# JSybrandt/HypergraphEmbedding

Measured on AMD Instinct MI355X. Metric: training samples/sec + alg-dist SpMV GB/s, HOBE dim=128 at 1/2/4/8 MI355X, higher is better.
Workload: dtype f32; 1 GPU; C3 HG2V_ALG_DIST (HOBE) dim=128, random 100k/50k, 1 step = 1 training epoch; nodes=100000, edges=50000, nnz=1999903, records_per_epoch=59999992, batch=256, dim=128, num_neighbors=5, num_samples=200, parallelism=single GPU

## Files before the change

### hypergraphembedding_amd/csrc/hgx_ctx.hip

```cpp
#include <algorithm>
#include <cstring>
#include <vector>

#include "hgx_internal.h"

int hgx_fail(hgx_ctx *ctx, int code, const char *fmt, ...) {
  if (ctx) {
    char buf[1024];
    va_list ap;
    va_start(ap, fmt);
    vsnprintf(buf, sizeof(buf), fmt, ap);
    va_end(ap);
    ctx->err = buf;
  }
  return code;
}

int hgx_ensure(hgx_ctx *ctx, DevBuf &b, size_t bytes) {
  if (bytes == 0) bytes = 16;
  if (b.bytes >= bytes) return HGX_OK;
  if (b.p) {
    hipFree(b.p);
    b.p = nullptr;
    b.bytes = 0;
// ... 86 lines not shown
  if (!ctx) return HGX_EINVAL;
  HGX_CHECK(ctx, key, HGX_EINVAL, "null tuning key");
  const std::string k(key);
  Tuning &t = ctx->tune;
  if (k == "sample_reject_w") {
    HGX_CHECK(ctx, value >= 0, HGX_EINVAL, "sample_reject_w must be >= 0");
    t.sample_reject_w = value;
  } else if (k == "sample_mode3_shift_e") {
    HGX_CHECK(ctx, value >= -10 && value <= 10, HGX_EINVAL,
              "sample_mode3_shift_e must be in [-10, 10]");
    t.sample_mode3_shift_e = (int)value;
  } else if (k == "sample_mode3_shift") {
    HGX_CHECK(ctx, value >= -10 && value <= 10, HGX_EINVAL,
              "sample_mode3_shift must be in [-10, 10]");
    t.sample_mode3_shift = (int)value;
  } else if (k == "sample_mode3") {
    HGX_CHECK(ctx, value >= 0 && value <= 2, HGX_EINVAL, "sample_mode3 must be 0, 1 or 2");
    t.sample_mode3 = (int)value;
  } else if (k == "train_fused") {
    HGX_CHECK(ctx, value == 0 || value == 1, HGX_EINVAL, "train_fused must be 0 or 1");
    t.train_fused = (int)value;
  } else if (k == "train_lanes") {
    HGX_CHECK(ctx, value == 0 || value == 32 || value == 64, HGX_EINVAL,
              "train_lanes must be 0, 32 or 64");
    t.train_lanes = (int)value;
  } else if (k == "train_tb") {
    HGX_CHECK(ctx, value == 0 || value == 128 || value == 256 || value == 512, HGX_EINVAL,
              "train_tb must be 0, 128, 256 or 512");
    t.train_tb = (int)value;
  } else if (k == "train_wave_pair") {
    HGX_CHECK(ctx, (value >= -1 && value <= 1) || value == 3 || value == 4, HGX_EINVAL,
              "train_wave_pair must be -1, 0, 1, 3 or 4");
    t.train_wave_pair = (int)value;
  } else if (k == "alg_long") {
    HGX_CHECK(ctx, value == 0 || (value >= 64 && value <= (1 << 20)), HGX_EINVAL,
              "alg_long must be 0 or in [64, 2^20]");
    t.alg_long = (int)value;
  } else if (k == "alg_push") {
    HGX_CHECK(ctx, value == 0 || value == 1, HGX_EINVAL, "alg_push must be 0 or 1");
    t.alg_push = (int)value;
  } else if (k == "mlp_fuse_head") {
    HGX_CHECK(ctx, value == 0 || value == 1, HGX_EINVAL, "mlp_fuse_head must be 0 or 1");
    t.mlp_fuse_head = (int)value;
  } else if (k == "mlp_prefetch") {
    HGX_CHECK(ctx, value >= 0 && value <= 2, HGX_EINVAL, "mlp_prefetch must be 0, 1 or 2");
    t.mlp_prefetch = (int)value;
  } else if (k == "mlp_wgrad_split") {
    HGX_CHECK(ctx, value >= 0 && value <= 1, HGX_EINVAL, "mlp_wgrad_split must be 0 or 1");
    t.mlp_wgrad_split = (int)value;
  } else if (k == "svc_lds_m") {
    HGX_CHECK(ctx, value == 64 || value == 128 || value == 192, HGX_EINVAL,
              "svc_lds_m must be 64, 128 or 192");
    t.svc_lds_m = (int)value;
  } else if (k == "ae_chunk_rows") {
    HGX_CHECK(ctx, value >= 0 && value <= (1 << 16), HGX_EINVAL,
              "ae_chunk_rows must be in [0, 65536]");
    t.ae_chunk_rows = (int)value;
  } else if (k == "n2v_expand_w") {
    HGX_CHECK(ctx, value >= 0 && value <= (1 << 20), HGX_EINVAL,
              "n2v_expand_w must be in [0, 2^20]");
    t.n2v_expand_w = (int)value;
  } else if (k == "n2v_chunk_walks") {
    HGX_CHECK(ctx, value >= 0 && value <= (1 << 16), HGX_EINVAL,
              "n2v_chunk_walks must be in [0, 65536]");
    t.n2v_chunk_walks = (int)value;
  } else if (k == "dw_hot_levels") {
// ... 199 lines not shown
```

### hypergraphembedding_amd/csrc/hgx_internal.h

```cpp
#pragma once

#include <hip/hip_runtime.h>

#include <cstdarg>
#include <cstdint>
#include <cstdio>
#include <cstdlib>
#include <string>
#include <vector>

#include "hgx.h"

struct DevBuf {
  void *p = nullptr;
  size_t bytes = 0;
  template <class T> T *as() const { return reinterpret_cast<T *>(p); }
};

struct LongRows {
  DevBuf seg;
  DevBuf off;
  DevBuf rows;
  DevBuf part;
  int nlong = 0, nseg = 0, thresh = 0;
};
constexpr int kLongRow = 512;

struct Tuning {
  int64_t sample_reject_w = 1 << 15;
  int sample_mode3 = 0;
  int sample_mode3_shift = 1;
  int sample_mode3_shift_e = 1;
  int train_fused = 1;
  int train_lanes = 0;
  int train_tb = 0;
  int train_wave_pair = -1;
  int alg_long = 0;
  int alg_ks = 0;
  int alg_push = 0;
  int mlp_fuse_head = 1;
  int mlp_prefetch = 1;
  int mlp_wgrad_split = 0;
  int train_prep_overlap = 0;
  int train_prep_cus = 0;
  int svc_lds_m = 128;
  int ae_chunk_rows = 0;
  int n2v_expand_w = 256;
  int n2v_chunk_walks = 0;
  int dw_hot_levels = 6;
};

struct hgx_ctx {
  int device = 0;
  hipStream_t stream = nullptr;
  hipStream_t own_stream = nullptr;
  std::string err;

  int32_t N = 0, E = 0;
  int64_t nnz = 0;
  uint64_t inc_gen = 0;
  DevBuf rp_n, col_n, rp_e, col_e;
  DevBuf blk_n, blk_e;
  int nblk_n = 0, nblk_e = 0;
  LongRows long_n, long_e;
  double avg_deg_n = 0, avg_deg_e = 0;
  int32_t max_deg_n = 0, max_deg_e = 0;

  int k = 0, ks = 0;
  DevBuf X[2], Y[2];
// ... 263 lines not shown
```

### hypergraphembedding_amd/csrc/hgx_train.hip

```cpp
#include <hipcub/hipcub.hpp>

#include <algorithm>
#include <cmath>
#include <cstdlib>
#include <cstring>
#include <vector>

#include "hgx_internal.h"
#include "hgx_train_common.h"
#include "hgx_train_split.h"
#include "hgx_train_step.h"
#include "hgx_train_prep.h"
#include "hgx_train_layout.h"

namespace {

int grid_for(int64_t work, int per_block) {
  int64_t g = (work + per_block - 1) / per_block;
  return (int)std::max<int64_t>(1, std::min<int64_t>(g, 4096));
}

void geometry(int d, int &L, int &VPL) {
  const int nv = (d + 3) / 4;
  L = 1;
// ... 37 lines not shown
using KStepFn = void (*)(TrainArgs, int, int, int, int);
#endif
using KFlushFn = void (*)(TrainArgs, const int *, const int *, const int *, int, int);

template <int SL, int VW, int TB>
void step_fns(int loss, KStepFn *kf, KFlushFn &kfl) {
  kf[0] = loss == 0 ? train_step<SL, VW, 5, 1, TB, false>
                    : train_step<SL, VW, 5, 2, TB, false>;
  kf[1] = loss == 0 ? train_step<SL, VW, 5, 1, TB, true>
                    : train_step<SL, VW, 5, 2, TB, true>;
  kfl = train_flush<SL * VW / 4>;
}
#ifndef HGX_TRAIN_CHUNKWAIT
#define HGX_TRAIN_CHUNKWAIT 0
#endif
constexpr bool kMergePair4 = HGX_TRAIN_ONEKERNEL >= 1;
constexpr bool kMergeAll = HGX_TRAIN_ONEKERNEL == 2;
template <int VW>
void step_fns_pair(int loss, KStepFn *kf, KFlushFn &kfl) {
  constexpr bool M0 = kMergeAll || (kMergePair4 && VW == 4);
  kf[0] = loss == 0 ? train_step<64, VW, 5, 1, 512, M0, true>
                    : train_step<64, VW, 5, 2, 512, M0, true>;
  kf[1] = loss == 0 ? train_step<64, VW, 5, 1, 512, true, true>
                    : train_step<64, VW, 5, 2, 512, true, true>;
  kfl = train_flush<64 * VW / 4>;
}
template <int RPB>
void step_fns_quad(int loss, KStepFn *kf, KFlushFn &kfl) {
  kf[0] = loss == 0 ? train_step_q<2, 5, 1, kMergeAll, RPB> : train_step_q<2, 5, 2, kMergeAll, RPB>;
  kf[1] = loss == 0 ? train_step_q<2, 5, 1, true, RPB> : train_step_q<2, 5, 2, true, RPB>;
  kfl = train_flush<32>;
}
constexpr int kPairDefault128 = 4, kPairDefault256 = 1;
bool pick_step(int L, int VPL, int K, int loss, int act, int lanes, int pair, int &sl,
               int &tb, int &rpb, KStepFn *kf, KFlushFn &kfl) {
  if (VPL != 1 || K != 5 || loss != act) return false;
  if (L != 32 && L != 64) return false;
  const int vw = L == 32 && lanes != 32 ? 2 : 4;
  sl = L * 4 / vw;
  const int pair_auto = tb != 0 ? 0 : vw == 2 ? kPairDefault128 : kPairDefault256;
  const int form = pair < 0 ? pair_auto : pair;
  if (sl == 64 && vw == 2 && form == 3) {
    tb = 512;
    rpb = 2;
    step_fns_quad<2>(loss, kf, kfl);
    return true;
  }
  if (sl == 64 && vw == 2 && form == 4) {
    tb = 256;
    rpb = 1;
    step_fns_quad<1>(loss, kf, kfl);
    return true;
  }
  if (sl == 64 && form) {
    tb = 512;
    rpb = 4;
    if (vw == 2) step_fns_pair<2>(loss, kf, kfl);
    else step_fns_pair<4>(loss, kf, kfl);
    return true;
  }
  if (sl == 32) {
    tb = tb == 256 ? 256 : 128;
    if (tb == 128) step_fns<32, 4, 128>(loss, kf, kfl);
    else step_fns<32, 4, 256>(loss, kf, kfl);
  } else if (vw == 2) {
    tb = tb == 512 || tb == 128 ? tb : 256;
// ... 293 lines not shown
  HGX_CHECK(ctx, max_epochs >= 0, HGX_EINVAL, "epochs must be >= 0");
  HGX_CHECK(ctx, loss == 0 || loss == 1, HGX_EINVAL, "loss must be 0 or 1");
  HGX_CHECK(ctx, act == 0 || act == 1, HGX_EINVAL, "act must be 0 or 1");
  HGX_CHECK(ctx, ctx->n_rec < (int64_t)INT32_MAX, HGX_EUNSUP, "more than 2^31 records");
  HGX_HIP(ctx, hipSetDevice(ctx->device));
  const int K = ctx->K, R = 4 + 2 * K;
  HGX_CHECK(ctx, (size_t)sort_slots(batch * R) * 8 <= 64 * 1024, HGX_EUNSUP,
            "batch_size*(4+2K)=%d exceeds the 8192-slot batch limit", batch * R);
  HGX_TRY(hgx_ensure(ctx, ctx->s0, 16));
  HGX_HIP(ctx, hipMemsetAsync(ctx->s0.p, 0, 16, ctx->stream));
  hipLaunchKernelGGL(max_index, dim3(grid_for(ctx->n_rec, 256)), dim3(256), 0, ctx->stream,
                     ctx->rec_idx.as<int>(), ctx->n_rec, R, K, ctx->s0.as<int>());
  HGX_LAUNCH_CHECK(ctx);
  int mx[4] = {0, 0, 0, 0};
  HGX_HIP(ctx, hipMemcpyAsync(mx, ctx->s0.p, 16, hipMemcpyDeviceToHost, ctx->stream));
  HGX_HIP(ctx, hipStreamSynchronize(ctx->stream));
  HGX_CHECK(ctx, mx[2] == 0, HGX_EINVAL, "negative record index");
  HGX_CHECK(ctx, mx[0] < ctx->node_rows && mx[1] < ctx->edge_rows, HGX_EINVAL,
            "record index (node %d, edge %d) outside the tables (%lld, %lld)",
            mx[0], mx[1], (long long)ctx->node_rows, (long long)ctx->edge_rows);
  return HGX_OK;
}

struct TrainPlan : hgx_layout::Dims {
  int64_t n, nbatches, nchunks;
  int K, SB, P, L, VPL;
  float lr, eps;
  int loss, act;
  int tb1, tb2, grid2;
  KFn k1 = nullptr, k2 = nullptr;
  KStepFn kf[2] = {nullptr, nullptr};
  KFlushFn kfl = nullptr;
  int tbf, lstride;
  bool ahead;
  size_t prep_smem, place_smem;
  int chunk_batches(int64_t c) const { return (int)std::min<int64_t>(CB, nbatches - c * CB); }
};

static int plan_split(hgx_ctx *ctx, TrainPlan &p) {
  p.tb1 = env_int("HGX_TRAIN_TB1", p.L >= 64 ? 512 : kTB);
  if (p.tb1 != 512) p.tb1 = kTB;
  if (!(p.K == 5 && p.loss == p.act) || env_int("HGX_TRAIN_GENERIC", 0) == 1) p.tb1 = kTB;
  p.tb2 = env_int("HGX_TRAIN_TB2", 512);
  if (p.tb2 != 512) p.tb2 = kTB;
  HGX_CHECK(ctx, pick_kernels(p.L, p.VPL, p.K, p.loss, p.act, p.tb1, p.tb2, p.k1, p.k2),
            HGX_EUNSUP, "no kernel for d=%d", ctx->d);
  p.RPB = p.tb1 / p.L;
  p.nblk1 = (p.batch + p.RPB - 1) / p.RPB;
  const int GPB2 = p.tb2 / p.L;
  p.grid2 = (p.SB + GPB2 - 1) / GPB2 + 2;
  return HGX_OK;
}

static int train_plan(hgx_ctx *ctx, int batch, float lr, float eps, int loss, int act,
                      TrainPlan &p) {
  p.n = ctx->n_rec;
  p.batch = batch, p.K = ctx->K, p.R = 4 + 2 * p.K, p.dp = ctx->dp, p.r0slots = kR0Slots;
  p.lr = lr, p.eps = eps, p.loss = loss, p.act = act;
  p.SB = batch * p.R;
  p.P = sort_slots(p.SB);
  geometry(ctx->d, p.L, p.VPL);
  HGX_TRY(plan_split(ctx, p));
  p.tbf = ctx->tune.train_tb;
  int SL = 0, rpbf = 0;
  p.fused = ctx->tune.train_fused && env_int("HGX_TRAIN_GENERIC", 0) != 1 && batch <= kPackB &&
            pick_step(p.L, p.VPL, p.K, loss, act, ctx->tune.train_lanes,
                      ctx->tune.train_wave_pair, SL, p.tbf, rpbf, p.kf, p.kfl);
  p.prpb = p.fused ? rpbf : 0;
  p.NBF = p.fused ? (batch + p.prpb - 1) / p.prpb : 0;
  p.RW = p.R + kWX;
  p.Mmax = p.SB / 2 + 1;
  p.MX = p.fused ? 2 + p.Mmax : 0;
  HGX_CHECK(ctx, p.MX <= (int)kDefMask + 1, HGX_EUNSUP, "batch too large for the step");
  const bool r0e = HGX_TRAIN_R0EARLY && p.fused && ctx->dp == 2 * SL;
  p.lstride = std::max(p.nblk1, r0e ? p.NBF * p.prpb : p.NBF);
  p.nbatches = (p.n + batch - 1) / batch;
  p.CB = (int)std::min<int64_t>(1024, (p.nbatches + kChunkRound - 1) / kChunkRound * kChunkRound);
  p.nchunks = (p.nbatches + p.CB - 1) / p.CB;
  p.overlap = p.fused && ctx->tune.train_prep_overlap >= 1;
  p.ahead = p.overlap && ctx->tune.train_prep_overlap == 2;
  p.prep_smem = p.P == kSortP ? ((size_t)p.P * 8 + std::max<size_t>(kPrepB * 4, (size_t)p.SB * 2) + 15) / 16 * 16
                              : (size_t)p.P * 12 + kPrepB * 4;
  p.place_smem = sizeof(int) * ((size_t)p.Mmax + p.SB);
  return HGX_OK;
}

struct TrainTrace {
  static constexpr int kBatches = 256;
  static constexpr size_t kBytes = sizeof(unsigned long long) * kBatches * 2 * 1024 * 8;
  const char *path = nullptr;
  void *p = nullptr;
  int begin(hgx_ctx *ctx) {
    path = hgx_debug_env_str("HGX_TRAIN_TRACE");
    if (path && path[0]) {
      HGX_HIP(ctx, hipMalloc(&p, kBytes));
      HGX_HIP(ctx, hipMemset(p, 0, kBytes));
    }
#ifdef HGX_DEBUG_KNOBS
    const int ab = env_int("HGX_TRAIN_ABLATE", 0), tn = p ? kBatches : 0;
    HGX_HIP(ctx, hipMemcpyToSymbol(HIP_SYMBOL(g_tab), &ab, sizeof(int)));
    HGX_HIP(ctx, hipMemcpyToSymbol(HIP_SYMBOL(g_trace), &p, sizeof(p)));
    HGX_HIP(ctx, hipMemcpyToSymbol(HIP_SYMBOL(g_trace_nb), &tn, sizeof(tn)));
#endif
    return HGX_OK;
  }
  void write_out() const {
    std::vector<unsigned long long> h(p ? kBytes / 8 : 0);
    if (!p || hipMemcpy(h.data(), p, kBytes, hipMemcpyDeviceToHost) != hipSuccess) return;
// ... 127 lines not shown
      }
      hbrk = ctx->train_hbrk;
    }
    if (p.overlap && !p.ahead) {
      HGX_TRY(train_streams(ctx, ctx->tune.train_prep_cus));
      sst = ctx->tstream[0];
      spr = ctx->tstream[1];
    }
    bev.assign(2 * p.nchunks, nullptr);
    pev.assign(p.overlap ? p.nchunks + 1 : 0, nullptr);
    for (auto &e : bev) HGX_HIP(ctx, hipEventCreate(&e));
    for (auto &e : pev) HGX_HIP(ctx, hipEventCreateWithFlags(&e, hipEventDisableTiming));
    return HGX_OK;
  }
  int set_of(int64_t c) const { return p.overlap ? (int)(c & 1) : 0; }

  void begin_epoch() {
    (void)hipMemsetAsync(dloss, 0, sizeof(double), ctx->stream);
    (void)hipMemsetAsync(ap[0].lossbuf, 0, sizeof(float) * (size_t)p.nbatches * p.lstride,
                         ctx->stream);
    if (p.fused) (void)hipMemsetAsync(ap[0].r0acc, 0, hgx_layout::r0acc_bytes(p), ctx->stream);
    if (p.overlap && !p.ahead) {
      (void)hipEventRecord(pev[p.nchunks], ctx->stream);
      (void)hipStreamWaitEvent(sst, pev[p.nchunks], 0);
      (void)hipStreamWaitEvent(spr, pev[p.nchunks], 0);
    }
  }
  void prepare(int64_t c) {
    const int nbc = p.chunk_batches(c), cp = (int)(c & 1), set = set_of(c);
    hipLaunchKernelGGL(train_prep, dim3(p.CB), dim3(kTB), p.prep_smem, spr, ap[0], c * p.CB, nbc,
                       p.P, skey[cp], sM[cp]);
    if (!p.fused) return;
    hipLaunchKernelGGL(train_place, dim3(p.CB), dim3(kTB), p.place_smem, spr, ap[set], nbc, p.CB,
                       skey[cp], sM[cp], skey[cp ^ 1], sM[cp ^ 1], c > 0 ? 1 : 0);
    if (!merged)
      flags_err = hipMemcpyAsync(hbrk + (size_t)set * p.CB, ap[set].pbrk, sizeof(int) * nbc,
                                 hipMemcpyDeviceToHost, spr);
    if (p.overlap) (void)hipEventRecord(pev[c], spr);
  }
  int wait_prepared(int64_t c) {
    hipError_t e = hipSuccess;
    if (p.overlap) {
      e = hipEventSynchronize(pev[c]);
      if (e == hipSuccess && !p.ahead) (void)hipStreamWaitEvent(sst, pev[c], 0);
    } else if (p.fused && !merged) {
      e = flags_err != hipSuccess ? flags_err : hipStreamSynchronize(spr);
    }
    if (e == hipSuccess) return HGX_OK;
    return hgx_fail(ctx, HGX_EHIP, "batch preparation failed: %s",
                    hipGetErrorString(hipGetLastError()));
  }
  void run_steps(int64_t c) {
    const int nbc = p.chunk_batches(c), set = set_of(c);
    for (int bi = 0; bi < nbc; bi++) {
      if (!p.fused) {
        hipLaunchKernelGGL(p.k1, dim3(p.nblk1), dim3(p.tb1), 0, sst, ap[0], bi);
        hipLaunchKernelGGL(p.k2, dim3(p.grid2), dim3(p.tb2), 0, sst, ap[0], bi);
        continue;
      }
      const int64_t gbat = c * p.CB + bi;
      const int nrec = (int)std::min<int64_t>(p.batch, p.n - gbat * p.batch);
      const int multi = merged || (hbrk[(size_t)set * p.CB + bi] && gbat > 0);
#if HGX_TRAIN_PRELOAD
      const TrainArgs &as = ap[set];
      const size_t g0 = (size_t)bi * p.NBF * p.prpb;
      hipLaunchKernelGGL(p.kf[multi], dim3(p.NBF), dim3(p.tbf), 0, sst, as.pidx + g0 * p.RW,
                         as.pcode + g0 * p.RW, as.ptgt + g0 * 3, p.RW, nrec, (int)gbat,
// ... 161 lines not shown
```

### hypergraphembedding_amd/csrc/hgx_train_prep.h

```cpp
#pragma once
#include <rocprim/block/block_radix_sort.hpp>

#include "hgx_train_step.h"

namespace {

__device__ int block_exclusive_scan(int v, int *total, int *s_ws) {
  const int lane = threadIdx.x & 63, wave = threadIdx.x >> 6;
  int inc = v;
#pragma unroll
  for (int off = 1; off < 64; off <<= 1) {
    const int o = __shfl_up(inc, off);
    if (lane >= off) inc += o;
  }
  if (lane == 63) s_ws[wave] = inc;
  __syncthreads();
  int base = 0, tot = 0;
  for (int w = 0; w < kTB / 64; w++) {
    if (w < wave) base += s_ws[w];
    tot += s_ws[w];
  }
  __syncthreads();
  *total = tot;
  return base + inc - v;
}

__device__ __forceinline__ int emit_pos(int s, int K) {
  if (s >= 4 + K) return 2 * (s - 4 - K) + 1;
  if (s >= 4) return 2 * (s - 4);
  return 2 * K + (s == 0 ? 0 : s == 3 ? 1 : s == 2 ? 2 : 3);
}

__device__ void defer_codes(const TrainArgs &a, int cb, int V, int P, int u0,
                            const unsigned long long *s_key, int *s_ws, int *s_runm,
                            int *skey, int *sM) {
// ... 162 lines not shown
    } else if (cur) {
      int rs = t;
      while (rs > 0 && k32(rs - 1) == kk[i]) rs--;
      int re = t + 1;
      while (re < V && k32(re) == kk[i]) re++;
      const int me = emit_pos(vv[i] % R, a.K);
      int first = 1, last = 1, own = vv[i] % R;
      for (int j = rs; j < re; j++) {
        const int e2 = emit_pos(slot(j) % R, a.K);
        first &= e2 >= me;
        last &= e2 <= me;
        if (e2 > emit_pos(own, a.K)) own = slot(j) % R;
      }
      code = kSLocal | (last ? kSOwn : 0u) | (first ? kSFirst : 0u) | (unsigned)own;
    }
    sc[vv[i]] = code;
  }
  if (threadIdx.x == 0) sM[cb] = S;
}

__device__ __forceinline__ int bsearch_lds(const int *v, int n, int key) {
  int lo = 0, hi = n;
  while (lo < hi) {
    const int mid = (lo + hi) >> 1;
    if (v[mid] < key) lo = mid + 1;
    else hi = mid;
  }
  return lo < n && v[lo] == key ? lo : -1;
}

__global__ __launch_bounds__(kTB) void train_place(TrainArgs a, int nbc, int CB,
                                                   const int *skey_cur, const int *sM_cur,
                                                   const int *skey_pc, const int *sM_pc,
                                                   int has_prev) {
  extern __shared__ int s_dyn[];
  __shared__ int s_pos[kPackB];
  __shared__ int s_ws[kTB / 64];
  const int cb = blockIdx.x;
  if (cb >= nbc) return;
  const int nb = a.bmeta[cb].x;
  const int R = a.R, K = a.K, RW = a.RW, RPB = a.prpb, SB = a.SB;
  const int G = (a.B + RPB - 1) / RPB * RPB;
  const int *prev = nullptr;
  int Mp = 0, Mpp = 0;
  if (cb > 0) {
    prev = skey_cur + (size_t)(cb - 1) * a.Mmax;
    Mp = sM_cur[cb - 1];
  } else if (has_prev) {
    prev = skey_pc + (size_t)(CB - 1) * a.Mmax;
    Mp = sM_pc[CB - 1];
  }
  if (cb > 1) Mpp = sM_cur[cb - 2];
  else if (has_prev) Mpp = sM_pc[CB - 2 + cb];
  const int U = a.ucount[cb];
  int *s_prev = s_dyn, *s_u = s_dyn + a.Mmax;
  __shared__ int s_brk;
  if (threadIdx.x == 0) s_brk = 0;
  for (int j = threadIdx.x; j < Mp; j += kTB) s_prev[j] = prev[j];
  for (int j = threadIdx.x; j < U; j += kTB) s_u[j] = a.ukey[(size_t)cb * SB + j];
  const int *bidx = a.bidx + (size_t)cb * a.B * R;
  const float *btgt = a.btgt + (size_t)cb * a.B * 3;
  __syncthreads();
  for (int i = threadIdx.x; i < nb && Mp; i += kTB) {
    int e0 = -1;
    for (int s2 = 0; s2 < R; s2++) {
      const int row = bidx[i * R + s2];
      if (row == 0) continue;
      const int j = bsearch_lds(s_prev, Mp, ((int)slot_is_edge(s2, K) << 30) | row);
      if (j < 0) continue;
      if (e0 >= 0 && j != e0) s_brk = 1;
      e0 = j;
    }
  }
  __syncthreads();
  if (threadIdx.x == 0) {
    a.pbrk[cb] = s_brk;
    if (s_brk) atomicAdd(a.ovf + kOvfMulti, 1);
  }
  {
    const int per = (nb + kTB - 1) / kTB, i0 = threadIdx.x * per, i1 = min(i0 + per, nb);
    int cs = 0;
    for (int i = i0; i < i1; i++) {
      int any = 0;
      for (int s = 4; s < R; s++) any |= bidx[i * R + s];
      s_pos[i] = any;
      cs += any == 0;
    }
    int NS = 0;
    int bs = block_exclusive_scan(cs, &NS, s_ws);
    const int NBF = G / RPB;
    for (int i = i0; i < i1; i++) {
      const bool sh = s_pos[i] == 0;
      const int p = sh ? bs : NS + (i - bs);
      s_pos[i] = (p % NBF) * RPB + p / NBF;
      bs += sh;
    }
  }
  int *pidx = a.pidx + (size_t)cb * G * RW;
  unsigned *pcode = a.pcode + (size_t)cb * G * RW;
  float *ptgt = a.ptgt + (size_t)cb * G * 3;
  for (int t = threadIdx.x; t < G * RW; t += kTB) {
    pidx[t] = 0;
    pcode[t] = 0u;
  }
  for (int t = threadIdx.x; t < G * 3; t += kTB) ptgt[t] = 0.f;
  __syncthreads();
  const unsigned *sc = a.scode + (size_t)cb * SB;
  for (int t = threadIdx.x; t < nb * R; t += kTB) {
    const int i = t / R, s = t - i * R;
    const int row = bidx[t];
    unsigned code = 0;
    if (row != 0) {
      code = sc[t];
      if (Mp) {
        const int j = bsearch_lds(s_prev, Mp, ((int)slot_is_edge(s, K) << 30) | row);
        if (j >= 0) code |= kSPend | ((unsigned)(2 + j) << kDefBits);
      }
    }
    pidx[s_pos[i] * RW + s] = row;
    pcode[s_pos[i] * RW + s] = code;
  }
  for (int t = threadIdx.x; t < nb * 3; t += kTB) {
    const int i = t / 3;
    ptgt[s_pos[i] * 3 + (t - 3 * i)] = btgt[t];
  }
  const int per = (Mp + kTB - 1) / kTB, j0 = threadIdx.x * per, j1 = min(j0 + per, Mp);
  int cf = 0;
  for (int j = j0; j < j1; j++) cf += bsearch_lds(s_u, U, s_prev[j]) < 0;
  int F = 0;
  int f = block_exclusive_scan(cf, &F, s_ws);
  const int cap = kFX * nb;
  for (int j = j0; j < j1; j++) {
    const int key = s_prev[j];
    if (bsearch_lds(s_u, U, key) >= 0) continue;
    if (f < cap) {
      const int p = f % nb, k = f / nb, g = (p % (G / RPB)) * RPB + p / (G / RPB);
      pidx[g * RW + R + k] = key & 0x3fffffff;
      pcode[g * RW + R + k] = ((key >> 30) ? kFEdge : 0u) | ((unsigned)(2 + j) << kDefBits);
    } else {
      a.pfo[(size_t)cb * a.Mmax + (f - cap)] = make_int2(key, 2 + j);
    }
    f++;
  }
  const int nfo = max(F - cap, 0);
  for (int g = threadIdx.x; g < G; g += kTB) {
    pidx[g * RW + R + kFX] = nfo;
    pidx[g * RW + R + kFX + 1] = Mpp;
  }
}

__global__ __launch_bounds__(kTB) void train_prep(TrainArgs a, int64_t base,
                                                  int nbc, int P, int *skey, int *sM) {
  extern __shared__ __attribute__((aligned(16))) unsigned long long s_key[];
  __shared__ int s_ws[kTB / 64];
  const int cb = blockIdx.x;
  if (cb >= nbc) {
    if (threadIdx.x == 0) a.bmeta[cb] = make_int2(0, 0);
    return;
  }
  unsigned long long ts[8] = {0, 0, 0, 0, 0, 0, 0, 0};
  if (g_trace) ts[0] = __builtin_amdgcn_s_memrealtime();
  const int64_t r0 = (base + cb) * a.B;
  const int nb = (int)min((int64_t)a.B, a.n - r0);
  if (threadIdx.x == 0) a.bmeta[cb] = make_int2(nb, (int)(base + cb));
  const int R = a.R, K = a.K;
  const int S = nb * R;
  int *bidx = a.bidx + (size_t)cb * a.B * R;
  float *btgt = a.btgt + (size_t)cb * a.B * 3;
  int *s_perm = reinterpret_cast<int *>(s_key + P) + (P == kSortP ? 0 : P);
  for (int i = threadIdx.x; i < nb; i += kTB) s_perm[i] = a.perm[r0 + i];
  __syncthreads();
  HGX_STAMP(ts[1]);
  for (int t = threadIdx.x; t < nb * 3; t += kTB) {
    const int i = t / 3;
    btgt[t] = a.tgt[(int64_t)s_perm[i] * 3 + (t - 3 * i)];
  }
  for (int t0 = threadIdx.x; t0 < P; t0 += 8 * kTB) {
    int rv[8];
#pragma unroll
    for (int u = 0; u < 8; u++) {
      const int t = t0 + u * kTB, i = t / R;
// ... 207 lines not shown
```

### hypergraphembedding_amd/csrc/hgx_train_step.h

```cpp
#pragma once
#include "hgx_divk.h"
#include "hgx_fix.h"
#include "hgx_train_split.h"

namespace {



#ifndef HGX_TRAIN_PRELOAD
#define HGX_TRAIN_PRELOAD 1
#endif
#ifndef HGX_TRAIN_HOSTINVB
#define HGX_TRAIN_HOSTINVB HGX_TRAIN_PRELOAD
#endif
struct StepWords {
  const int *pidx;
  const unsigned *pcode;
  const float *ptgt;
  int RW;
  float inv_b;
};
#if HGX_TRAIN_PRELOAD
#define HGX_STEP_PARAMS                                                              \
  const int *w_pidx, const unsigned *w_pcode, const float *w_ptgt, int w_rw, int nb, \
      int q, float w_inv_b, int gb, int cb, TrainArgs a
#define HGX_STEP_WORDS(RPB)                                \
  const StepWords w = {w_pidx, w_pcode, w_ptgt, w_rw,      \
                       HGX_TRAIN_HOSTINVB ? w_inv_b : 1.0f / (float)nb}
#else
#define HGX_STEP_PARAMS TrainArgs a, int cb, int gb, int nb, int q
#define HGX_STEP_WORDS(RPB)                                                       \
  const size_t w_g0 = (size_t)cb * gridDim.x * (RPB);                             \
  const StepWords w = {a.pidx + w_g0 * a.RW, a.pcode + w_g0 * a.RW, a.ptgt + w_g0 * 3, \
                       a.RW, 1.0f / (float)nb}
#endif
// ... 246 lines not shown
  __shared__ float s_loss[RPB];
  __shared__ float s_x[RPB][4];
  unsigned long long ts[8] = {0, 0, 0, 0, 0, 0, 0, 0};
  if (g_trace) ts[0] = __builtin_amdgcn_s_memrealtime();
  const int wave = __builtin_amdgcn_readfirstlane(threadIdx.x / L), lane = threadIdx.x % L;
  const int grp = wave >> 1, half = wave & 1;
  const bool edge = half;
  const int NBF = gridDim.x, RW = w.RW;
  const int par = q % 3, ppar = (q + 2) % 3, zpar = (q + 1) % 3;
  const unsigned gi = blockIdx.x * RPB + grp;
  const int *ri = w.pidx + gi * RW;
  const unsigned *rc = w.pcode + gi * RW;
  const float *yt = w.ptgt + gi * 3;
  const int sl = lane < RW ? lane : 0;
  const int rv = ri[sl];
  const int cv = (int)rc[sl];
  const int tv = __float_as_int(yt[lane < 3 ? lane : 0]);
  Row0Loads<L, VW> r0l;
  if (wave < 2) row0_issue<L, VW>(a, q, r0l);
  int row[J], frow[kFX];
  unsigned code[J], fcode[kFX];
  const int sH = edge ? 3 : 0, sO = edge ? 1 : 2, sT = 4 + half * K;
  auto slot_of = [&](int j) { return j == 0 ? sH : j == 1 ? sO : sT + j - 2; };
#pragma unroll
  for (int j = 0; j < J; j++) {
    row[j] = __builtin_amdgcn_readlane(rv, slot_of(j));
    code[j] = (unsigned)__builtin_amdgcn_readlane(cv, slot_of(j));
  }
#pragma unroll
  for (int f = 0; f < kFX; f++) {
    frow[f] = __builtin_amdgcn_readlane(rv, R + f);
    fcode[f] = (unsigned)__builtin_amdgcn_readlane(cv, R + f);
  }
  const int nfo = __builtin_amdgcn_readlane(rv, R + kFX);
  const int zc = __builtin_amdgcn_readlane(rv, R + kFX + 1);
  const float yt0 = __int_as_float(__builtin_amdgcn_readlane(tv, 0));
  const float yt1 = __int_as_float(__builtin_amdgcn_readlane(tv, 1));
  const float yt2 = __int_as_float(__builtin_amdgcn_readlane(tv, 2));
  HGX_STAMP(ts[1]);
  const int nval = min(max(nb - (int)blockIdx.x + NBF - 1, 0) / NBF, RPB);
  const bool has = grp < nval;
  int bad = 0;
  if (nval > 0) {
    V *Tw = reinterpret_cast<V *>(edge ? a.etab : a.ntab);
    V *Aw = reinterpret_cast<V *>(edge ? a.eacc : a.nacc);
    const V *T = Tw, *Ac = Aw;
    V Pv[J], Av[J];
    bool lists = false;
#pragma unroll
    for (int j = 2; j < J; j++) lists |= row[j] != 0;
    auto gather = [&](int j) {
      const int arow = (code[j] & kSOwn) ? row[j] : 0;
      Pv[j] = T[(size_t)row[j] * L + lane];
      Av[j] = Ac[(size_t)arow * L + lane];
    };
#pragma unroll
    for (int j = 0; j < 2; j++) {
      if (row[j] == 0) {
        Pv[j] = Av[j] = S::zero();
        continue;
      }
      gather(j);
    }
    if (lists) {
#pragma unroll
      for (int j = 2; j < J; j++) gather(j);
    }
// ... 130 lines not shown
            S::adagrad(pv, av, S::add(*acc, g), a.lr, a.eps);
            st_row(&Tw[(size_t)row[j] * L + lane], pv);
            st_row(&Aw[(size_t)row[j] * L + lane], av);
          } else {
            *acc = (cd & kSFirst) ? g : S::add(*acc, g);
          }
        } else if (cd & kSShared) {
          const int m = cd & kDefMask;
          S::addfix(gacc_row<L, VW>(a, par, m), lane, g, bad);
          if (cd & kSOwn) {
            st_row(&sh_row<L, VW>(a, par, m, 0)[lane], Pv[j]);
            st_row(&sh_row<L, VW>(a, par, m, 1)[lane], Av[j]);
          }
        } else {
          V pv = Pv[j], av = Av[j];
          S::adagrad(pv, av, g, a.lr, a.eps);
          st_row(&Tw[(size_t)row[j] * L + lane], pv);
          st_row(&Aw[(size_t)row[j] * L + lane], av);
        }
      };
      V gH = S::fma(dz, O, S::zero());
      if (kR0E) {
        float d[K];
#pragma unroll
        for (int k = 0; k < K; k++) {
          d[k] = dk * act_d_nc(act, zk[k], sk[k]);
          gH = S::fma(d[k], Pv[2 + k], gH);
          if (row[2 + k] == 0) zT = S::add(zT, S::fma(d[k], H, S::zero()));
        }
        if (row[0] == 0) zT = S::add(zT, gH);
        if (row[1] == 0) zT = S::add(zT, S::fma(dz, H, S::zero()));
        const int slot = (blockIdx.x * RPB + grp) % R0S<VW * L>::n;
        S::addfix(r0_row<L, VW>(a, par, slot, half), lane, zT, bad);
        if (!edge && lane == 0)
          a.lossbuf[(size_t)gb * a.lstride + blockIdx.x * RPB + grp] = lrec;
#pragma unroll
        for (int k = 0; k < K; k++) emit(2 + k, S::fma(d[k], H, S::zero()));
      } else {
#pragma unroll
        for (int k = 0; k < K; k++) {
          const float d = dk * act_d_nc(act, zk[k], sk[k]);
          gH = S::fma(d, Pv[2 + k], gH);
          emit(2 + k, S::fma(d, H, S::zero()));
        }
      }
      emit(0, gH);
      emit(1, S::fma(dz, H, S::zero()));
      HGX_STAMP(ts[4]);
    }
    if (!kR0E) {
      s_z[half][grp][lane] = zT;
      if (!edge && lane == 0) s_loss[grp] = lrec;
      __syncthreads();
      if (wave < 2) {
        V sz = S::zero();
        for (int g = 0; g < RPB; g++) sz = S::add(sz, s_z[wave][g][lane]);
        S::addfix(r0_row<L, VW>(a, par, blockIdx.x % R0S<VW * L>::n, wave), lane, sz, bad);
      }
      if (threadIdx.x == 0) {
        float sl = 0.f;
        for (int g = 0; g < RPB; g++) sl += s_loss[g];
        a.lossbuf[(size_t)gb * a.lstride + blockIdx.x] = sl;
      }
    }
#pragma unroll
    for (int f = 1; f < kFX; f++)
      if (frow[f] != 0 && (f & 1) == half) flush_slot<L, VW>(a, ppar, frow[f], fcode[f], lane);
  }
// ... 48 lines not shown
  __shared__ V s_t[RPB][2][KL][L];
  __shared__ __attribute__((aligned(16))) float s_zx[RPB][2][8];
  unsigned long long ts[8] = {0, 0, 0, 0, 0, 0, 0, 0};
  if (g_trace) ts[0] = __builtin_amdgcn_s_memrealtime();
  const int wave = __builtin_amdgcn_readfirstlane(threadIdx.x / L), lane = threadIdx.x % L;
  const int grp = wave >> 2, half = (wave >> 1) & 1, sub = wave & 1;
  const bool edge = half;
  const int NBF = gridDim.x, RW = w.RW;
  const int par = q % 3, ppar = (q + 2) % 3, zpar = (q + 1) % 3;
  const unsigned gi = blockIdx.x * RPB + grp;
  const int *ri = w.pidx + gi * RW;
  const unsigned *rc = w.pcode + gi * RW;
  const float *yt = w.ptgt + gi * 3;
  const int sl = lane < RW ? lane : 0;
  const int rv = ri[sl];
  const int cv = (int)rc[sl];
  const int tv = __float_as_int(yt[lane < 3 ? lane : 0]);
  Row0Loads<L, VW> r0l;
  if (wave < 2) row0_issue<L, VW>(a, q, r0l);
  int row[J], frow[kFX];
  unsigned code[J], fcode[kFX];
  const int sH = edge ? 3 : 0, sO = edge ? 1 : 2, sT = 4 + half * K;
  auto slot_of = [&](int j) { return j == 0 ? sH : j == 1 ? sO : sT + j - 2; };
#pragma unroll
  for (int j = 0; j < J; j++) {
    row[j] = __builtin_amdgcn_readlane(rv, slot_of(j));
    code[j] = (unsigned)__builtin_amdgcn_readlane(cv, slot_of(j));
  }
#pragma unroll
  for (int f = 0; f < kFX; f++) {
    frow[f] = __builtin_amdgcn_readlane(rv, R + f);
    fcode[f] = (unsigned)__builtin_amdgcn_readlane(cv, R + f);
  }
  const int nfo = __builtin_amdgcn_readlane(rv, R + kFX);
  const int zc = __builtin_amdgcn_readlane(rv, R + kFX + 1);
  const float yt0 = __int_as_float(__builtin_amdgcn_readlane(tv, 0));
  const float yt1 = __int_as_float(__builtin_amdgcn_readlane(tv, 1));
  const float yt2 = __int_as_float(__builtin_amdgcn_readlane(tv, 2));
  HGX_STAMP(ts[1]);
  const int nval = min(max(nb - (int)blockIdx.x + NBF - 1, 0) / NBF, RPB);
  const bool has = grp < nval;
  unsigned lc = 0;
#pragma unroll
  for (int j = JH; j < J; j++) lc |= code[j];
  const bool split = !(lc & kSLocal);
  const int role = !has ? kQIdle : sub == 0 ? (split ? kQHead : kQFull) : (split ? kQList : kQIdle);
  auto by_role = [&](auto &&f) __attribute__((always_inline)) {
    if (role == kQHead) f(QC<kQHead>{});
    else if (role == kQList) f(QC<kQList>{});
    else if (role == kQFull) f(QC<kQFull>{});
  };
  int bad = 0;
  if (nval > 0) {
    V *Tw = reinterpret_cast<V *>(edge ? a.etab : a.ntab);
    V *Aw = reinterpret_cast<V *>(edge ? a.eacc : a.nacc);
    const V *T = Tw, *Ac = Aw;
    V Pv[J], Av[J];
    by_role([&](auto rl) __attribute__((always_inline)) {
      using QR = QRole<decltype(rl)::value, J, JH>;
      bool lists = false;
#pragma unroll
      for (int j = 2; j < J; j++)
        if ((QR::pm >> j) & 1u) lists |= row[j] != 0;
#pragma unroll
      for (int j = 0; j < J; j++) {
        if (!((QR::pm >> j) & 1u)) continue;
        if (j < 2 ? row[j] != 0 : lists) {
// ... 153 lines not shown
          }
        } else if (cd & kSShared) {
          const int m = cd & kDefMask;
          S::addfix(gacc_row<L, VW>(a, par, m), lane, g, bad);
          if (cd & kSOwn) {
            st_row(&sh_row<L, VW>(a, par, m, 0)[lane], Pv[j]);
            st_row(&sh_row<L, VW>(a, par, m, 1)[lane], Av[j]);
          }
        } else {
          V pv = Pv[j], av = Av[j];
          S::adagrad(pv, av, g, a.lr, a.eps);
          st_row(&Tw[(size_t)row[j] * L + lane], pv);
          st_row(&Aw[(size_t)row[j] * L + lane], av);
        }
      };
      float d[K];
#pragma unroll
      for (int k = 0; k < K; k++) d[k] = dk * act_d_nc(act, zk[k], sk[k]);
      if (ROLE != kQList) {
        if (ROLE == kQHead) {
#pragma unroll
          for (int k = KH; k < K; k++) Pv[2 + k] = s_t[grp][half][k - KH][lane];
        }
        V gH = S::fma(dz, O, S::zero()), zT = S::zero();
#pragma unroll
        for (int k = 0; k < K; k++) {
          gH = S::fma(d[k], Pv[2 + k], gH);
          if (row[2 + k] == 0) zT = S::add(zT, S::fma(d[k], H, S::zero()));
        }
        if (row[0] == 0) zT = S::add(zT, gH);
        if (row[1] == 0) zT = S::add(zT, S::fma(dz, H, S::zero()));
        const int slot = (blockIdx.x * RPB + grp) % R0S<VW * L>::n;
        S::addfix(r0_row<L, VW>(a, par, slot, half), lane, zT, bad);
        if (!edge && lane == 0)
          a.lossbuf[(size_t)gb * a.lstride + blockIdx.x * RPB + grp] = lrec;
#pragma unroll
        for (int k = 0; k < K; k++)
          if ((QR::om >> (2 + k)) & 1u) emit(2 + k, S::fma(d[k], H, S::zero()));
        emit(0, gH);
        emit(1, S::fma(dz, H, S::zero()));
      } else {
#pragma unroll
        for (int k = KH; k < K; k++) emit(2 + k, S::fma(d[k], H, S::zero()));
      }
      HGX_STAMP(ts[4]);
    });
#pragma unroll
    for (int f = 1; f < kFX; f++)
      if (frow[f] != 0 && f == (wave & 3)) flush_slot<L, VW>(a, ppar, frow[f], fcode[f], lane);
  }
  HGX_STAMP(ts[5]);
  for (int e = blockIdx.x * NW + wave; e < nfo; e += NBF * NW) {
    const int2 en = a.pfo[(size_t)cb * a.Mmax + e];
    flush_row<L, VW>(a, ppar, en.x, en.y, lane);
  }
  {
    longlong2 *z = reinterpret_cast<longlong2 *>(gacc_row<L, VW>(a, zpar, 2));
    const int tot = zc * (VW / 2) * L;
    for (int i = blockIdx.x * TB + threadIdx.x; i < tot; i += NBF * TB)
      z[i] = make_longlong2(0, 0);
    longlong2 *zr = reinterpret_cast<longlong2 *>(r0_row<L, VW>(a, zpar, 0, 0));
    for (int i = blockIdx.x * TB + threadIdx.x; i < R0S<VW * L>::n * VW * L; i += NBF * TB)
      zr[i] = make_longlong2(0, 0);
  }
  if (__any(bad) && !g_tab && lane == 0) atomicOr(a.ovf, 1);
  HGX_STAMP(ts[6]);
  trace_put(gb, 0, 7, ts, threadIdx.x == (NW - 4) * L);
}

template <int VW, int KMAX, int MODE, bool MULTI, int RPB>
__global__ __launch_bounds__(256 * RPB) void train_step_q(HGX_STEP_PARAMS) {
  HGX_STEP_WORDS(RPB);
  train_step_quad<VW, KMAX, MODE, MULTI, RPB>(a, w, cb, gb, nb, q);
}

template <int L, int VW, int KMAX, int MODE, int TB, bool MULTI, bool PAIR = false>
__global__ __launch_bounds__(TB) void train_step(HGX_STEP_PARAMS) {
  HGX_STEP_WORDS(PAIR ? 4 : TB / L);
  if constexpr (PAIR) {
    static_assert(!PAIR || (L == 64 && TB == 512), "paired geometry");
    train_step_pair<VW, KMAX, MODE, MULTI>(a, w, cb, gb, nb, q);
    return;
  }
  constexpr int RPB = TB / L, R = 4 + 2 * KMAX, K = KMAX, NC = 2 * L;
  using S = SV<VW>;
  using V = typename S::T;
  static_assert(L == 32 || L == 64, "step geometry");
  static_assert(R + kWX <= 32, "slot and batch words fit the first 32 lanes");
  constexpr bool kR0E = HGX_TRAIN_R0EARLY && VW == 2;
  __shared__ V s_z[2][RPB][L];
  __shared__ V s_gl[RPB][R][L];
  __shared__ V s_r0[2][L];
  __shared__ float s_loss[RPB];
  unsigned long long ts[8] = {0, 0, 0, 0, 0, 0, 0, 0};
  if (g_trace) ts[0] = __builtin_amdgcn_s_memrealtime();
  const int grp = threadIdx.x / L, lane = threadIdx.x % L;
  const int NBF = gridDim.x, RW = w.RW;
  const int par = q % 3, ppar = (q + 2) % 3, zpar = (q + 1) % 3;
  const unsigned gi = blockIdx.x * RPB + grp;
  const int *ri = w.pidx + gi * RW;
  const unsigned *rc = w.pcode + gi * RW;
  const float *yt = w.ptgt + gi * 3;
  int row[R], frow[kFX];
  unsigned code[R], fcode[kFX];
  int nfo, zc;
  const int sl = lane < RW ? lane : 0;
  const int rv = ri[sl];
  const int cv = (int)rc[sl];
  const int tv = __float_as_int(yt[L == 64 ? (lane < 3 ? lane : 0) : 0]);
  float yt1 = 0.f, yt2 = 0.f;
  if (L == 32) {
    yt1 = yt[1];
    yt2 = yt[2];
  }
  Row0Loads<L, VW> r0l;
  row0_issue<L, VW>(a, q, r0l);
  {
#pragma unroll
    for (int s = 0; s < R + kFX; s++) {
      int r, c;
      if (L == 64) {
        r = __builtin_amdgcn_readlane(rv, s);
        c = __builtin_amdgcn_readlane(cv, s);
      } else {
        const bool hi = threadIdx.x & 32;
        const int r0 = __builtin_amdgcn_readlane(rv, s), r1 = __builtin_amdgcn_readlane(rv, 32 + s);
        const int c0 = __builtin_amdgcn_readlane(cv, s), c1 = __builtin_amdgcn_readlane(cv, 32 + s);
        r = hi ? r1 : r0;
        c = hi ? c1 : c0;
      }
      if (s < R) {
        row[s] = r;
        code[s] = (unsigned)c;
      } else {
        frow[s - R] = r;
        fcode[s - R] = (unsigned)c;
      }
    }
    nfo = __builtin_amdgcn_readlane(rv, R + kFX);
    zc = __builtin_amdgcn_readlane(rv, R + kFX + 1);
  }
  float yt0 = __int_as_float(tv);
  if (L == 64) {
    yt0 = __int_as_float(__builtin_amdgcn_readlane(tv, 0));
    yt1 = __int_as_float(__builtin_amdgcn_readlane(tv, 1));
    yt2 = __int_as_float(__builtin_amdgcn_readlane(tv, 2));
  }
  HGX_STAMP(ts[1]);
  const int nval = min(max(nb - (int)blockIdx.x + NBF - 1, 0) / NBF, RPB);
  const bool has = grp < nval;
  const int col = threadIdx.x % NC, sub = threadIdx.x / NC, tab0 = col / L, c0 = col % L;
  int bad = 0;
  if (nval > 0) {
    V p0 = r0l.rp, a0 = r0l.ra;
    S::pin(p0);
    S::pin(a0);
    V Pv[R], Av[R];
    bool lists = false;
#pragma unroll
    for (int s = 4; s < R; s++) lists |= row[s] != 0;
    const bool wave_lists = __any(lists);
    auto gather = [&](int s) {
      const bool edge = slot_is_edge(s, K);
      const V *T = reinterpret_cast<const V *>(edge ? a.etab : a.ntab);
      const V *Ac = reinterpret_cast<const V *>(edge ? a.eacc : a.nacc);
      const int arow = (code[s] & kSOwn) ? row[s] : 0;
      Pv[s] = T[(size_t)row[s] * L + lane];
      Av[s] = Ac[(size_t)arow * L + lane];
    };
#pragma unroll
    for (int s = 0; s < 4; s++) {
      if (L == 64 && row[s] == 0) {
// ... 178 lines not shown
            st_row(&sh_row<L, VW>(a, par, m, 1)[lane], Av[s]);
          }
        } else {
          V pv = Pv[s], av = Av[s];
          if (g_tab & 8192) {
            pv = S::add(pv, g);
            av = S::add(av, g);
          } else {
            S::adagrad(pv, av, g, a.lr, a.eps);
          }
          st_row(&tab_row<L, VW>(a, edge, 0, row[s])[lane], pv);
          st_row(&tab_row<L, VW>(a, edge, 1, row[s])[lane], av);
        }
      };
      V gln = S::fma(dz1, Nr, S::zero()), gre = S::fma(dz2, El, S::zero());
      if (kR0E) {
        float da[K], db[K];
#pragma unroll
        for (int k = 0; k < K; k++) {
          da[k] = dP * act_d_nc(act, za[k], sa[k]);
          db[k] = dQ * act_d_nc(act, zb[k], sb[k]);
          gln = S::fma(da[k], Pv[4 + k], gln);
          gre = S::fma(db[k], Pv[4 + K + k], gre);
          if (row[4 + k] == 0) zN = S::add(zN, S::fma(da[k], Nl, S::zero()));
          if (row[4 + K + k] == 0) zE = S::add(zE, S::fma(db[k], Er, S::zero()));
        }
        if (row[0] == 0) zN = S::add(zN, gln);
        if (row[3] == 0) zE = S::add(zE, gre);
        if (row[2] == 0) zN = S::add(zN, S::fma(dz1, Nl, S::zero()));
        if (row[1] == 0) zE = S::add(zE, S::fma(dz2, Er, S::zero()));
        const int slot = (blockIdx.x * RPB + grp) % R0S<VW * L>::n;
        S::addfix(r0_row<L, VW>(a, par, slot, 0), lane, zN, bad);
        S::addfix(r0_row<L, VW>(a, par, slot, 1), lane, zE, bad);
        if (lane == 0) a.lossbuf[(size_t)gb * a.lstride + blockIdx.x * RPB + grp] = lrec;
#pragma unroll
        for (int k = 0; k < K; k++) {
          emit(4 + k, S::fma(da[k], Nl, S::zero()));
          emit(4 + K + k, S::fma(db[k], Er, S::zero()));
        }
      } else {
#pragma unroll
        for (int k = 0; k < K; k++) {
          const float da = dP * act_d_nc(act, za[k], sa[k]);
          const float db = dQ * act_d_nc(act, zb[k], sb[k]);
          gln = S::fma(da, Pv[4 + k], gln);
          gre = S::fma(db, Pv[4 + K + k], gre);
          emit(4 + k, S::fma(da, Nl, S::zero()));
          emit(4 + K + k, S::fma(db, Er, S::zero()));
        }
      }
      emit(0, gln);
      emit(3, gre);
      emit(2, S::fma(dz1, Nl, S::zero()));
      emit(1, S::fma(dz2, Er, S::zero()));
      HGX_STAMP(ts[4]);
    }
    if (!kR0E) {
      s_z[0][grp][lane] = zN;
      s_z[1][grp][lane] = zE;
      if (lane == 0) s_loss[grp] = lrec;
      if (!(g_tab & 16384)) __syncthreads();
      if (threadIdx.x < NC && !(g_tab & 16384)) {
        V sz = S::zero();
        for (int g = 0; g < RPB; g++) sz = S::add(sz, s_z[tab0][g][c0]);
        S::addfix(r0_row<L, VW>(a, par, blockIdx.x % R0S<VW * L>::n, tab0), c0, sz, bad);
      }
      if (threadIdx.x == 0) {
// ... 64 lines not shown
```

Baseline: 46.52 million records/s.

## Order record placement by pending-dependency class to reduce step-kernel stalls

```diff
diff --git a/hypergraphembedding_amd/csrc/hgx_ctx.hip b/hypergraphembedding_amd/csrc/hgx_ctx.hip
--- a/hypergraphembedding_amd/csrc/hgx_ctx.hip
+++ b/hypergraphembedding_amd/csrc/hgx_ctx.hip
@@ -142,6 +142,10 @@
     HGX_CHECK(ctx, (value >= -1 && value <= 1) || value == 3 || value == 4, HGX_EINVAL,
               "train_wave_pair must be -1, 0, 1, 3 or 4");
     t.train_wave_pair = (int)value;
+  } else if (k == "train_place_order") {
+    HGX_CHECK(ctx, value >= -1 && value <= 1, HGX_EINVAL,
+              "train_place_order must be -1, 0 or 1");
+    t.train_place_order = (int)value;
   } else if (k == "alg_long") {
     HGX_CHECK(ctx, value == 0 || (value >= 64 && value <= (1 << 20)), HGX_EINVAL,
               "alg_long must be 0 or in [64, 2^20]");
diff --git a/hypergraphembedding_amd/csrc/hgx_internal.h b/hypergraphembedding_amd/csrc/hgx_internal.h
--- a/hypergraphembedding_amd/csrc/hgx_internal.h
+++ b/hypergraphembedding_amd/csrc/hgx_internal.h
@@ -35,6 +35,7 @@
   int train_lanes = 0;
   int train_tb = 0;
   int train_wave_pair = -1;
+  int train_place_order = -1;
   int alg_long = 0;
   int alg_ks = 0;
   int alg_push = 0;
diff --git a/hypergraphembedding_amd/csrc/hgx_place_order.h b/hypergraphembedding_amd/csrc/hgx_place_order.h
--- /dev/null
+++ b/hypergraphembedding_amd/csrc/hgx_place_order.h
@@ -0,0 +1,21 @@
+#pragma once
+
+#if defined(__HIPCC__) || defined(__CUDACC__)
+#define HGX_PLACE_HD __host__ __device__ __forceinline__
+#else
+#define HGX_PLACE_HD inline
+#endif
+
+HGX_PLACE_HD int place_class(bool has_pending, bool has_list) {
+  return has_pending ? 0 : has_list ? 1 : 2;
+}
+
+HGX_PLACE_HD int place_position(int order, int cls, bool has_list, int rank_cls, int rank_list,
+                                int n0, int n1, int ns) {
+  if (order == 0) return has_list ? ns + rank_list : rank_list;
+  return (cls == 0 ? 0 : cls == 1 ? n0 : n0 + n1) + rank_cls;
+}
+
+HGX_PLACE_HD int flush_position(int order, int f, int nb) {
+  return order == 0 ? f % nb : nb - 1 - f % nb;
+}
diff --git a/hypergraphembedding_amd/csrc/hgx_train.hip b/hypergraphembedding_amd/csrc/hgx_train.hip
--- a/hypergraphembedding_amd/csrc/hgx_train.hip
+++ b/hypergraphembedding_amd/csrc/hgx_train.hip
@@ -93,6 +93,7 @@
   kfl = train_flush<32>;
 }
 constexpr int kPairDefault128 = 4, kPairDefault256 = 1;
+constexpr bool kPlaceOrderDefault1 = true;
 bool pick_step(int L, int VPL, int K, int loss, int act, int lanes, int pair, int &sl,
                int &tb, int &rpb, KStepFn *kf, KFlushFn &kfl) {
   if (VPL != 1 || K != 5 || loss != act) return false;
@@ -452,6 +453,7 @@
   KStepFn kf[2] = {nullptr, nullptr};
   KFlushFn kfl = nullptr;
   int tbf, lstride;
+  int order = 0;
   bool ahead;
   size_t prep_smem, place_smem;
   int chunk_batches(int64_t c) const { return (int)std::min<int64_t>(CB, nbatches - c * CB); }
@@ -494,6 +496,12 @@
   HGX_CHECK(ctx, p.MX <= (int)kDefMask + 1, HGX_EUNSUP, "batch too large for the step");
   const bool r0e = HGX_TRAIN_R0EARLY && p.fused && ctx->dp == 2 * SL;
   p.lstride = std::max(p.nblk1, r0e ? p.NBF * p.prpb : p.NBF);
+  p.order = ctx->tune.train_place_order;
+  HGX_CHECK(ctx, !(p.fused && p.order == 1 && !r0e), HGX_EUNSUP,
+            "train_place_order 1 needs float2 rows (d <= 128): at float4 rows the padding "
+            "row's gradient is a float sum over the workgroup's records, and moving records "
+            "between workgroups would change its bits");
+  if (p.order < 0) p.order = kPlaceOrderDefault1 && r0e && p.prpb == 1 ? 1 : 0;
   p.nbatches = (p.n + batch - 1) / batch;
   p.CB = (int)std::min<int64_t>(1024, (p.nbatches + kChunkRound - 1) / kChunkRound * kChunkRound);
   p.nchunks = (p.nbatches + p.CB - 1) / p.CB;
@@ -687,7 +695,7 @@
                        p.P, skey[cp], sM[cp]);
     if (!p.fused) return;
     hipLaunchKernelGGL(train_place, dim3(p.CB), dim3(kTB), p.place_smem, spr, ap[set], nbc, p.CB,
-                       skey[cp], sM[cp], skey[cp ^ 1], sM[cp ^ 1], c > 0 ? 1 : 0);
+                       skey[cp], sM[cp], skey[cp ^ 1], sM[cp ^ 1], c > 0 ? 1 : 0, p.order);
     if (!merged)
       flags_err = hipMemcpyAsync(hbrk + (size_t)set * p.CB, ap[set].pbrk, sizeof(int) * nbc,
                                  hipMemcpyDeviceToHost, spr);
diff --git a/hypergraphembedding_amd/csrc/hgx_train_prep.h b/hypergraphembedding_amd/csrc/hgx_train_prep.h
--- a/hypergraphembedding_amd/csrc/hgx_train_prep.h
+++ b/hypergraphembedding_amd/csrc/hgx_train_prep.h
@@ -1,6 +1,7 @@
 #pragma once
 #include <rocprim/block/block_radix_sort.hpp>
 
+#include "hgx_place_order.h"
 #include "hgx_train_step.h"
 
 namespace {
@@ -229,7 +230,7 @@
 __global__ __launch_bounds__(kTB) void train_place(TrainArgs a, int nbc, int CB,
                                                    const int *skey_cur, const int *sM_cur,
                                                    const int *skey_pc, const int *sM_pc,
-                                                   int has_prev) {
+                                                   int has_prev, int order) {
   extern __shared__ int s_dyn[];
   __shared__ int s_pos[kPackB];
   __shared__ int s_ws[kTB / 64];
@@ -258,9 +259,9 @@
   const int *bidx = a.bidx + (size_t)cb * a.B * R;
   const float *btgt = a.btgt + (size_t)cb * a.B * 3;
   __syncthreads();
-  for (int i = threadIdx.x; i < nb && Mp; i += kTB) {
+  for (int i = threadIdx.x; i < nb; i += kTB) {
     int e0 = -1;
-    for (int s2 = 0; s2 < R; s2++) {
+    for (int s2 = 0; s2 < R && Mp; s2++) {
       const int row = bidx[i * R + s2];
       if (row == 0) continue;
       const int j = bsearch_lds(s_prev, Mp, ((int)slot_is_edge(s2, K) << 30) | row);
@@ -268,29 +269,41 @@
       if (e0 >= 0 && j != e0) s_brk = 1;
       e0 = j;
     }
+    s_pos[i] = e0 >= 0;
   }
   __syncthreads();
   if (threadIdx.x == 0) {
     a.pbrk[cb] = s_brk;
     if (s_brk) atomicAdd(a.ovf + kOvfMulti, 1);
   }
+  const int NBF = G / RPB;
+  auto group_of = [&](int p) { return (p % NBF) * RPB + p / NBF; };
   {
+    static_assert(kPackB < (1 << 10), "three counts packed in one scan");
     const int per = (nb + kTB - 1) / kTB, i0 = threadIdx.x * per, i1 = min(i0 + per, nb);
     int cs = 0;
     for (int i = i0; i < i1; i++) {
       int any = 0;
       for (int s = 4; s < R; s++) any |= bidx[i * R + s];
-      s_pos[i] = any;
-      cs += any == 0;
-    }
-    int NS = 0;
-    int bs = block_exclusive_scan(cs, &NS, s_ws);
-    const int NBF = G / RPB;
+      const int cls = place_class(s_pos[i] != 0, any != 0);
+      s_pos[i] = cls | (any != 0) << 2;
+      cs += (any == 0) | (cls == 0) << 10 | (cls == 1) << 20;
+    }
+    int tot = 0;
+    const int bs = block_exclusive_scan(cs, &tot, s_ws);
+    const int NS = tot & 1023, N0 = (tot >> 10) & 1023, N1 = tot >> 20;
+    int rs = bs & 1023, r0 = (bs >> 10) & 1023, r1 = bs >> 20;
     for (int i = i0; i < i1; i++) {
-      const bool sh = s_pos[i] == 0;
-      const int p = sh ? bs : NS + (i - bs);
-      s_pos[i] = (p % NBF) * RPB + p / NBF;
-      bs += sh;
+      const int cls = s_pos[i] & 3;
+      const bool list = s_pos[i] >> 2;
+      const int rl = list ? i - rs : rs;
+      const int rc = cls == 0 ? r0 : cls == 1 ? r1 : i - r0 - r1;
+      const int p0 = place_position(0, cls, list, rc, rl, N0, N1, NS);
+      const int p = order == 0 ? p0 : place_position(order, cls, list, rc, rl, N0, N1, NS);
+      s_pos[i] = group_of(p) | group_of(p0) << 16;
+      rs += !list;
+      r0 += cls == 0;
+      r1 += cls == 1;
     }
   }
   int *pidx = a.pidx + (size_t)cb * G * RW;
@@ -314,12 +327,13 @@
         if (j >= 0) code |= kSPend | ((unsigned)(2 + j) << kDefBits);
       }
     }
-    pidx[s_pos[i] * RW + s] = row;
-    pcode[s_pos[i] * RW + s] = code;
+    const int g = s_pos[i] & 0xffff;
+    pidx[g * RW + s] = row;
+    pcode[g * RW + s] = code;
   }
   for (int t = threadIdx.x; t < nb * 3; t += kTB) {
     const int i = t / 3;
-    ptgt[s_pos[i] * 3 + (t - 3 * i)] = btgt[t];
+    ptgt[(s_pos[i] & 0xffff) * 3 + (t - 3 * i)] = btgt[t];
   }
   const int per = (Mp + kTB - 1) / kTB, j0 = threadIdx.x * per, j1 = min(j0 + per, Mp);
   int cf = 0;
@@ -331,7 +345,7 @@
     const int key = s_prev[j];
     if (bsearch_lds(s_u, U, key) >= 0) continue;
     if (f < cap) {
-      const int p = f % nb, k = f / nb, g = (p % (G / RPB)) * RPB + p / (G / RPB);
+      const int k = f / nb, g = group_of(flush_position(order, f, nb));
       pidx[g * RW + R + k] = key & 0x3fffffff;
       pcode[g * RW + R + k] = ((key >> 30) ? kFEdge : 0u) | ((unsigned)(2 + j) << kDefBits);
     } else {
@@ -341,9 +355,11 @@
   }
   const int nfo = max(F - cap, 0);
   for (int g = threadIdx.x; g < G; g += kTB) {
-    pidx[g * RW + R + kFX] = nfo;
+    if ((g % RPB) * NBF + g / RPB >= nb) pidx[g * RW + R + kFX] = nfo;
     pidx[g * RW + R + kFX + 1] = Mpp;
   }
+  for (int i = threadIdx.x; i < nb; i += kTB)
+    pidx[(s_pos[i] & 0xffff) * RW + R + kFX] = nfo | (s_pos[i] >> 16) << 16;
 }
 
 __global__ __launch_bounds__(kTB) void train_prep(TrainArgs a, int64_t base,
diff --git a/hypergraphembedding_amd/csrc/hgx_train_step.h b/hypergraphembedding_amd/csrc/hgx_train_step.h
--- a/hypergraphembedding_amd/csrc/hgx_train_step.h
+++ b/hypergraphembedding_amd/csrc/hgx_train_step.h
@@ -1,6 +1,7 @@
 #pragma once
 #include "hgx_divk.h"
 #include "hgx_fix.h"
+#include "hgx_place_order.h"
 #include "hgx_train_split.h"
 
 namespace {
@@ -313,7 +314,8 @@
     frow[f] = __builtin_amdgcn_readlane(rv, R + f);
     fcode[f] = (unsigned)__builtin_amdgcn_readlane(cv, R + f);
   }
-  const int nfo = __builtin_amdgcn_readlane(rv, R + kFX);
+  const unsigned bw = (unsigned)__builtin_amdgcn_readlane(rv, R + kFX);
+  const int nfo = bw & 0xffffu, lpos = bw >> 16;
   const int zc = __builtin_amdgcn_readlane(rv, R + kFX + 1);
   const float yt0 = __int_as_float(__builtin_amdgcn_readlane(tv, 0));
   const float yt1 = __int_as_float(__builtin_amdgcn_readlane(tv, 1));
@@ -510,8 +512,7 @@
         if (row[1] == 0) zT = S::add(zT, S::fma(dz, H, S::zero()));
         const int slot = (blockIdx.x * RPB + grp) % R0S<VW * L>::n;
         S::addfix(r0_row<L, VW>(a, par, slot, half), lane, zT, bad);
-        if (!edge && lane == 0)
-          a.lossbuf[(size_t)gb * a.lstride + blockIdx.x * RPB + grp] = lrec;
+        if (!edge && lane == 0) a.lossbuf[(size_t)gb * a.lstride + lpos] = lrec;
 #pragma unroll
         for (int k = 0; k < K; k++) emit(2 + k, S::fma(d[k], H, S::zero()));
       } else {
@@ -626,7 +627,8 @@
     frow[f] = __builtin_amdgcn_readlane(rv, R + f);
     fcode[f] = (unsigned)__builtin_amdgcn_readlane(cv, R + f);
   }
-  const int nfo = __builtin_amdgcn_readlane(rv, R + kFX);
+  const unsigned bw = (unsigned)__builtin_amdgcn_readlane(rv, R + kFX);
+  const int nfo = bw & 0xffffu, lpos = bw >> 16;
   const int zc = __builtin_amdgcn_readlane(rv, R + kFX + 1);
   const float yt0 = __int_as_float(__builtin_amdgcn_readlane(tv, 0));
   const float yt1 = __int_as_float(__builtin_amdgcn_readlane(tv, 1));
@@ -846,8 +848,7 @@
         if (row[1] == 0) zT = S::add(zT, S::fma(dz, H, S::zero()));
         const int slot = (blockIdx.x * RPB + grp) % R0S<VW * L>::n;
         S::addfix(r0_row<L, VW>(a, par, slot, half), lane, zT, bad);
-        if (!edge && lane == 0)
-          a.lossbuf[(size_t)gb * a.lstride + blockIdx.x * RPB + grp] = lrec;
+        if (!edge && lane == 0) a.lossbuf[(size_t)gb * a.lstride + lpos] = lrec;
 #pragma unroll
         for (int k = 0; k < K; k++)
           if ((QR::om >> (2 + k)) & 1u) emit(2 + k, S::fma(d[k], H, S::zero()));
@@ -879,7 +880,12 @@
   }
   if (__any(bad) && !g_tab && lane == 0) atomicOr(a.ovf, 1);
   HGX_STAMP(ts[6]);
-  trace_put(gb, 0, 7, ts, threadIdx.x == (NW - 4) * L);
+  if (g_trace) {
+    const bool pend = __any(lane < R && ((unsigned)cv & kSPend));
+    const bool list = __any(lane >= 4 && lane < R && rv != 0);
+    ts[7] = 1 + place_class(pend, list);
+  }
+  trace_put(gb, 0, 8, ts, threadIdx.x == (NW - 4) * L);
 }
 
 template <int VW, int KMAX, int MODE, bool MULTI, int RPB>
@@ -918,6 +924,8 @@
   int row[R], frow[kFX];
   unsigned code[R], fcode[kFX];
   int nfo, zc;
+  int lpos;
+  static_assert(!(kR0E && L == 32), "one loss word per wave: 64 lanes per record");
   const int sl = lane < RW ? lane : 0;
   const int rv = ri[sl];
   const int cv = (int)rc[sl];
@@ -951,7 +959,8 @@
         fcode[s - R] = (unsigned)c;
       }
     }
-    nfo = __builtin_amdgcn_readlane(rv, R + kFX);
+    const unsigned bw = (unsigned)__builtin_amdgcn_readlane(rv, R + kFX);
+    nfo = bw & 0xffffu, lpos = bw >> 16;
     zc = __builtin_amdgcn_readlane(rv, R + kFX + 1);
   }
   float yt0 = __int_as_float(tv);
@@ -1196,7 +1205,7 @@
         const int slot = (blockIdx.x * RPB + grp) % R0S<VW * L>::n;
         S::addfix(r0_row<L, VW>(a, par, slot, 0), lane, zN, bad);
         S::addfix(r0_row<L, VW>(a, par, slot, 1), lane, zE, bad);
-        if (lane == 0) a.lossbuf[(size_t)gb * a.lstride + blockIdx.x * RPB + grp] = lrec;
+        if (lane == 0) a.lossbuf[(size_t)gb * a.lstride + lpos] = lrec;
 #pragma unroll
         for (int k = 0; k < K; k++) {
           emit(4 + k, S::fma(da[k], Nl, S::zero()));
```

Measured after the change: 46.66 million records/s, median of 3. No clear change (+0.3%).
